# perrysou/SoftGNSS-python

Hardware: NVIDIA B200
Metric: tracking channel-ms/s (higher is better)
Workload: dtype int8 x Q38 fixed-point correlators (exact int32 dot products), f64 rotors / accumulation / loop filters

## Files before the change

### softgnss_python_b200/csrc/sgx_common.cuh

```cuda
#pragma once
#include <stdint.h>
#include <stdio.h>
#include <string.h>
#include <mutex>

#ifdef SGX_EMUL
#include "cuda_emul.h"
#else
#include <cuda_runtime.h>
#define SGX_LAUNCH(kernel, grid, block, smem, stream, ...) \
  kernel<<<(grid), (block), (smem), (stream)>>>(__VA_ARGS__)
#define SGX_DYN_SMEM(name) extern __shared__ __align__(1024) unsigned char name[]
#endif

#include "../../include/softgnss_b200.h"

#ifdef SGX_EMUL
#define SGX_TABLE static
#else
#define SGX_TABLE static __constant__
#endif

namespace sgx {

// ... 91 lines not shown

__device__ __forceinline__ void mbar_init(unsigned long long* bar, unsigned count) {
#ifdef SGX_EMUL
  *bar = 0;
  (void)count;
#else
  unsigned s = (unsigned)__cvta_generic_to_shared(bar);
  asm volatile("mbarrier.init.shared::cta.b64 [%0], %1;\n" ::"r"(s), "r"(count) : "memory");
  asm volatile("fence.mbarrier_init.release.cluster;\n" ::: "memory");
#endif
}
__device__ __forceinline__ unsigned smem_addr(const void* p) {
#ifdef SGX_EMUL
  (void)p; return 0u;
#else
  unsigned a = (unsigned)__cvta_generic_to_shared(p), o;
  asm volatile("mov.u32 %0, %1;" : "=r"(o) : "r"(a));
  return o;
#endif
}
__device__ __forceinline__ unsigned lds_u32(const void* base, unsigned base_s, int byte_off) {
#ifdef SGX_EMUL
  (void)base_s; return *reinterpret_cast<const unsigned*>(reinterpret_cast<const char*>(base) + byte_off);
#else
  (void)base; unsigned v;
  asm volatile("ld.shared.u32 %0, [%1];" : "=r"(v) : "r"(base_s + (unsigned)byte_off));
  return v;
#endif
}
__device__ __forceinline__ uint4 lds_u32x4(const void* base, unsigned base_s, int byte_off) {
#ifdef SGX_EMUL
  (void)base_s; return *reinterpret_cast<const uint4*>(reinterpret_cast<const char*>(base) + byte_off);
#else
  (void)base; uint4 v;
  asm volatile("ld.shared.v4.u32 {%0, %1, %2, %3}, [%4];" : "=r"(v.x), "=r"(v.y), "=r"(v.z), "=r"(v.w)
               : "r"(base_s + (unsigned)byte_off));
  return v;
#endif
}
__device__ __forceinline__ double2 lds_f64x2(const void* base, unsigned base_s, int byte_off) {
#ifdef SGX_EMUL
  (void)base_s; return *reinterpret_cast<const double2*>(reinterpret_cast<const char*>(base) + byte_off);
#else
  (void)base; double2 v;
  asm volatile("ld.shared.v2.f64 {%0, %1}, [%2];" : "=d"(v.x), "=d"(v.y) : "r"(base_s + (unsigned)byte_off));
  return v;
#endif
}

__device__ __forceinline__ void bulk_load(void* smem_dst, const void* gsrc, unsigned bytes,
                                          unsigned long long* bar) {
#ifdef SGX_EMUL
  memcpy(smem_dst, gsrc, bytes);
  *bar += 1;
#else
  unsigned d = (unsigned)__cvta_generic_to_shared(smem_dst);
  unsigned b = (unsigned)__cvta_generic_to_shared(bar);
  asm volatile("mbarrier.arrive.expect_tx.shared::cta.b64 _, [%0], %1;\n" ::"r"(b), "r"(bytes) : "memory");
  asm volatile(
      "cp.async.bulk.shared::cluster.global.mbarrier::complete_tx::bytes [%0], [%1], %2, [%3];\n" ::"r"(d),
      "l"(gsrc), "r"(bytes), "r"(b)
      : "memory");
#endif
}
__device__ __forceinline__ void mbar_wait(unsigned long long* bar, unsigned parity) {
#ifdef SGX_EMUL
  while ((*(volatile unsigned long long*)bar & 1ull) == (unsigned long long)parity) sgx_emul::yield_to_sched();
#else
  unsigned b = (unsigned)__cvta_generic_to_shared(bar);
  asm volatile(
      "{\n"
      ".reg .pred p;\n"
      "LAB_WAIT:\n"
      "mbarrier.try_wait.parity.shared::cta.b64 p, [%0], %1;\n"
      "@p bra DONE;\n"
      "bra LAB_WAIT;\n"
      "DONE:\n"
      "}\n" ::"r"(b),
      "r"(parity)
      : "memory");
#endif
}

__device__ __forceinline__ float warp_sum(float v) {
#pragma unroll
  for (int m = 16; m > 0; m >>= 1) v += __shfl_xor_sync(0xffffffffu, v, m);
  return v;
}

__device__ __forceinline__ double warp_sum_f64(double v) {
#pragma unroll
  for (int m = 16; m > 0; m >>= 1) v += __shfl_xor_sync(0xffffffffu, v, m);
  return v;
}

}
```

### softgnss_python_b200/csrc/sgx_track.cu

```cuda
#include <vector>
#include <fcntl.h>
#include <sys/stat.h>
#include <unistd.h>
#include "sgx_common.cuh"

namespace sgx {

constexpr int TRK_THREADS = 256;
constexpr int TRK_WARPS = TRK_THREADS / 32;
constexpr int TRK_MARGIN = 256;
constexpr int TRK_PROF_N = 5;

struct TrackArgs {
  const int8_t* rec;
  long long rec_stride;
  const long long* rec_len;
  const sgx_channel* ch;
  const int8_t* chips;
  double* out;
  int* ms_done;
  int* status;
  int n_channels;
  int ms;
  int resume;
  long long avail;
  struct TrackState* state;
  long long* prof;
  int win;
  long long skip;
  long long abs_base;
  double fs, codeFreqBasis, codeLength, spc;
  double c1code, c2code, c1carr, c2carr;
};

struct MsParams {
  double startE, stepE, startL, stepL, startP, stepP;
  double inv_step;
  long long q0_fix, h_fix;
  double cps;
  double rem_cyc;
  double w;
  double rem_rad;
  double fs;
  long long pos;
  int blk;
  int stop;
};

__device__ __forceinline__ double lin_y(int i, double step, double start) {
  return __dadd_rn(__dmul_rn((double)i, step), start);
}

__device__ __forceinline__ int next_event(int c, double start, double step, double inv) {
  double q = ((double)c - start) * inv;
  double fl = floor(q);
  int i = (int)fl + 1;
  double fr = q - fl;
  if (fr < 1e-6 || fr > 1.0 - 1e-6) {
    while (i > 0 && lin_y(i - 1, step, start) > (double)c) --i;
    while (!(lin_y(i, step, start) > (double)c)) ++i;
  }
  return i;
}

struct CodeVar {
  double start, step;
  int c;
  int e;
  float s;
  __device__ __forceinline__ void init(int i0, double st, double sp, double inv, const float* code) {
    start = st;
    step = sp;
    c = (int)ceil(lin_y(i0, step, start));
    s = code[c];
    e = next_event(c, start, step, inv);
  }
  __device__ __forceinline__ void advance(double inv, const float* code) {
    c += 1;
    s = code[c];
    e = next_event(c, start, step, inv);
  }
};

__device__ __forceinline__ float byte_to_float(unsigned u_offset_binary, int k) {
  unsigned r = __byte_perm(u_offset_binary, 0x4B000000u, 0x7540u + (unsigned)k);
  return __uint_as_float(r) - 8388736.0f;
}

__device__ __forceinline__ void cis_cycles(double cyc, float& c, float& s) {
  cyc -= rint(cyc);
  const float hi = (float)cyc;
  const float lo = (float)(cyc - (double)hi) * 6.2831853071795865f;
  float s0, c0;
  sincospif(2.0f * hi, &s0, &c0);
  c = fmaf(-s0, lo, c0);
  s = fmaf(c0, lo, s0);
}

__device__ __forceinline__ void cmul(float& r, float& i, float ar, float ai, float br, float bi) {
  r = fmaf(ar, br, -(ai * bi));
  i = fmaf(ar, bi, ai * br);
}

struct CodeState {
  double codeFreq, remCodePhase, oldCodeNco, oldCodeError, nextRemCode;
  long long pos;
};
struct CarrState {
  double carrFreq, carrFreqBasis, remCarrPhase, oldCarrNco, oldCarrError, w;
};

constexpr int SGX_PAUSED = 1;

struct TrackState {
  CodeState c;
  CarrState r;
  int k;
  int status;
};

__device__ void prepare_code(const TrackArgs& a, CodeState& st, long long rec_len, MsParams& p, int lane) {
  const double step = st.codeFreq / a.fs;
  const double q = (lane == 1 ? 1.0 : a.codeLength - st.remCodePhase) / step;
  const int blk = (int)ceil(__shfl_sync(0xffffffffu, q, 0));
  const double inv_step = __shfl_sync(0xffffffffu, q, 1);
  const long long aligned = st.pos & ~15LL;
  int stop = 0;
  if (st.pos + blk > rec_len) stop = SGX_ERR_SHORT;
  else if (st.pos + blk > a.avail) stop = SGX_PAUSED;
  else if (blk <= 0 || (st.pos - aligned) + blk > a.win) stop = SGX_ERR_RANGE;
  if (lane == 0) { p.blk = blk; p.pos = st.pos; p.stop = stop; }
  if (stop) return;
  const double rem = st.remCodePhase, spc = a.spc, bs = (double)blk * step;
  const double startE = rem - spc, startL = rem + spc, startP = rem;
  const double num = lane == 0 ? ((bs + rem) - spc) - startE : lane == 1 ? ((bs + rem) + spc) - startL : (bs + rem) - startP;
  const double d = num / (double)blk;
  const double stepE = __shfl_sync(0xffffffffu, d, 0), stepL = __shfl_sync(0xffffffffu, d, 1),
               stepP = __shfl_sync(0xffffffffu, d, 2);
  if (lane == 0) {
    p.startE = startE; p.stepE = stepE;
    p.startL = startL; p.stepL = stepL;
    p.startP = startP; p.stepP = stepP;
    p.inv_step = inv_step;
    p.h_fix = __double2ll_rn(0.5 * inv_step * 1099511627776.0);
    p.q0_fix = __double2ll_rn(-rem * inv_step * 1099511627776.0);
  }
  st.nextRemCode = (lin_y(blk - 1, stepP, startP) + step) - 1023.0;
}

__device__ double prepare_carr(const TrackArgs& a, CarrState& st, MsParams& p, bool write) {
  st.w = st.carrFreq * 2.0 * 3.141592653589793;
  const double cps = (st.w / a.fs) * 0.15915494309189535;
  if (write) {
    p.cps = cps;
    p.w = st.w;
    p.fs = a.fs;
  }
  return cps;
}

__device__ __forceinline__ void set_carr_phase(MsParams& p, double rem) {
  p.rem_cyc = rem * 0.15915494309189535;
  p.rem_rad = rem;
}

__device__ double carry_carr_phase(double w, double rem, int blk, double fs) {
  const double TWO_PI = 6.283185307179586;
  double arg_end = w * ((double)blk / fs) + rem;
  double m;
  if (arg_end >= 0.0) {
    double q = floor(arg_end * 0.15915494309189535);
    m = __fma_rn(-q, TWO_PI, arg_end);
    if (m < 0.0) { q -= 1.0; m = __fma_rn(-q, TWO_PI, arg_end); }
    else if (m >= TWO_PI) { q += 1.0; m = __fma_rn(-q, TWO_PI, arg_end); }
  } else {
    m = fmod(arg_end, TWO_PI);
    if (m != 0.0 && m < 0.0) m += TWO_PI;
  }
  return m;
}

__device__ __forceinline__ void correlate_groups(const MsParams& P, const int8_t* cur, const float* codeS, int tid,
                                                 double& tEr, double& tEi, double& tPr, double& tPi, double& tLr,
                                                 double& tLi) {
    const int off = (int)(P.pos - (P.pos & ~15LL));
    const int ng = (off + P.blk + 15) >> 4;
    const int gpt = (ng + TRK_THREADS - 1) / TRK_THREADS;
    const int g0 = tid * gpt;
    const int g1 = min(g0 + gpt, ng);
    if (g0 < g1) {
      int ib = 16 * g0 - off;
      const int i0 = max(ib, 0);
      CodeVar E, Pm, L;
      E.init(i0, P.startE, P.stepE, P.inv_step, codeS);
      Pm.init(i0, P.startP, P.stepP, P.inv_step, codeS);
      L.init(i0, P.startL, P.stepL, P.inv_step, codeS);
      float wr[16], wi[16], w16r, w16i, rotr, roti;
      {
        cis_cycles((double)ib * P.cps + P.rem_cyc, rotr, roti);
        float s1, c1;
        cis_cycles(P.cps, c1, s1);
        wr[0] = 1.f; wi[0] = 0.f; wr[1] = c1; wi[1] = s1;
#pragma unroll
        for (int q = 2; q < 16; ++q) {
          cmul(wr[q], wi[q], wr[q >> 1], wi[q >> 1], wr[q - (q >> 1)], wi[q - (q >> 1)]);
        }
        cis_cycles(16.0 * P.cps, w16r, w16i);
      }
      for (int g = g0; g < g1; ++g, ib += 16) {
        uint4 q4 = *reinterpret_cast<const uint4*>(cur + 16 * g);
        unsigned wq[4] = {q4.x, q4.y, q4.z, q4.w};
        if (ib < 0 || ib + 16 > P.blk) {
#pragma unroll
          for (int b = 0; b < 16; ++b) {
            int i = ib + b;
            if (i < 0 || i >= P.blk) wq[b >> 2] &= ~(0xFFu << (8 * (b & 3)));
          }
        }
#pragma unroll
        for (int j = 0; j < 4; ++j) wq[j] ^= 0x80808080u;
        const int kE = E.e - ib, kP = Pm.e - ib, kL = L.e - ib;
// ... 175 lines not shown
        cmul(tr, ti, cr, ci, zr[4], zi[4]);
        cr = tr; ci = ti;
      }
    }
    float Rr, Ri;
    cmul(Rr, Ri, rotr, roti, Sr, Si);
    fEr = fmaf(sE, Rr, fEr); fEi = fmaf(sE, Ri, fEi);
    fPr = fmaf(sP, Rr, fPr); fPi = fmaf(sP, Ri, fPi);
    fLr = fmaf(sL, Rr, fLr); fLi = fmaf(sL, Ri, fLi);
    const int len = b - a0;
    const int j = len - (LMAX - 4);
    if (j >= 0 && j <= 4) {
      float sr = zr[0], si = zi[0];
      if (j == 1) { sr = zr[1]; si = zi[1]; }
      if (j == 2) { sr = zr[2]; si = zi[2]; }
      if (j == 3) { sr = zr[3]; si = zi[3]; }
      if (j == 4) { sr = zr[4]; si = zi[4]; }
      float nr, ni;
      cmul(nr, ni, rotr, roti, sr, si);
      rotr = nr; roti = ni;
    } else {
      fresh = true;
    }
  }
  tEr += (double)fEr; tEi += (double)fEi; tPr += (double)fPr; tPi += (double)fPi; tLr += (double)fLr; tLi += (double)fLi;
}

template <int NW> struct ExactDigits { static constexpr int value = NW <= 5 ? 5 : 4; };
struct __align__(16) ExactTables {
  signed char tw[2][5][32];
  double z[5][2];
};

__device__ __forceinline__ void sincos_reduced(double th, double& sn, double& cs) {
  const double k = rint(th * 0.6366197723675814);
  double r = fma(-k, 1.5707963267341256, th);
  r = fma(-k, 6.077100506303966e-11, r);
  r = fma(-k, 2.0222662487959506e-21, r);
  const double r2 = r * r;
  double ps = -7.647163731819816e-13;
  ps = fma(ps, r2, 1.6059043836821613e-10);
  ps = fma(ps, r2, -2.505210838544172e-08);
  ps = fma(ps, r2, 2.7557319223985893e-06);
  ps = fma(ps, r2, -1.984126984126984e-04);
  ps = fma(ps, r2, 8.333333333333333e-03);
  ps = fma(ps, r2, -1.6666666666666666e-01);
  const double s0 = fma(ps * r2, r, r);
  double pc = 4.779477332387385e-14;
  pc = fma(pc, r2, -1.1470745597729725e-11);
  pc = fma(pc, r2, 2.08767569878681e-09);
  pc = fma(pc, r2, -2.755731922398589e-07);
  pc = fma(pc, r2, 2.48015873015873e-05);
  pc = fma(pc, r2, -1.388888888888889e-03);
  pc = fma(pc, r2, 4.1666666666666664e-02);
  pc = fma(pc, r2, -0.5);
  const double c0 = fma(pc, r2, 1.0);
  const int q = (int)(long long)k & 3;
  const double sa = (q & 1) ? c0 : s0, ca = (q & 1) ? s0 : c0;
  sn = (q & 2) ? -sa : sa;
  cs = ((q + 1) & 2) ? -ca : ca;
}

__device__ __forceinline__ void cis_cycles_f64(double cyc, double& c, double& s) {
  cyc -= rint(cyc);
  sincospi(2.0 * cyc, &s, &c);
}

template <int NW>
__device__ __forceinline__ void build_exact_tables(ExactTables& T, double cps, int lane) {
  constexpr int LMAX = 4 * NW;
  constexpr int ND = ExactDigits<NW>::value;
  constexpr int Z0 = (LMAX + 5 <= 32) ? LMAX : 0;
  const bool tw = lane < LMAX, zs = lane >= Z0 && lane < Z0 + 5;
  if (tw || (Z0 > 0 && zs)) {
    double c, s;
    cis_cycles_f64((double)(tw ? lane : LMAX - 4 + (lane - Z0)) * cps, c, s);
    if (!tw) {
      T.z[lane - Z0][0] = c;
      T.z[lane - Z0][1] = s;
      return;
    }
    const double one = (double)(1LL << (8 * ND - 2));
    long long w[2] = {__double2ll_rn(c * one), __double2ll_rn(s * one)};
#pragma unroll
    for (int q = 0; q < 2; ++q) {
      long long v = w[q];
#pragma unroll
      for (int d = 0; d < ND - 1; ++d) {
        const long long b = ((v + 128) & 0xFF) - 128;
        T.tw[q][d][lane] = (signed char)b;
        v = (v - b) >> 8;
      }
      T.tw[q][ND - 1][lane] = (signed char)v;
    }
  }
  if (Z0 == 0 && zs) cis_cycles_f64((double)(LMAX - 4 + lane) * cps, T.z[lane][0], T.z[lane][1]);
}

constexpr int IRREGULAR = 1 << 30;
__device__ __noinline__ int settle_boundary(int n, const MsParams& P) {
  if ((n & 1) == 0) return max(0, min(next_event(n >> 1, P.startP, P.stepP, P.inv_step), P.blk));
  const int c = (n - 1) >> 1;
  const int b = next_event(c, P.startE, P.stepE, P.inv_step);
  const int bl = next_event(c + 1, P.startL, P.stepL, P.inv_step);
  return max(0, min(b, P.blk)) | (bl != b ? IRREGULAR : 0);
}

__device__ __noinline__ double2 start_rotor(int a, const MsParams& P) {
  const double th = P.w * ((double)a / P.fs) + P.rem_rad;
  double sn, cs;
  if (fabs(th) < 5.0e5) sincos_reduced(th, sn, cs);
  else sincos(th, &sn, &cs);
  return make_double2(cs, sn);
}

__device__ __noinline__ void correlate_per_sample(const MsParams& P, const int8_t* cur, const unsigned char* codeB, int off,
                                                  int i0, int i1, double* acc) {
  for (int i = i0; i < i1; ++i) {
    const int ie = (int)ceil(lin_y(i, P.stepE, P.startE));
    const int ip = (int)ceil(lin_y(i, P.stepP, P.startP));
    const int il = (int)ceil(lin_y(i, P.stepL, P.startL));
    double cs, sn;
    cis_cycles_f64((double)i * P.cps + P.rem_cyc, cs, sn);
    const double x = (double)cur[off + i];
    const double pr = x * cs, pi = x * sn;
    const double ce = codeB[ie] ? -1.0 : 1.0, cp = codeB[ip] ? -1.0 : 1.0, cl = codeB[il] ? -1.0 : 1.0;
    acc[0] += ce * pr; acc[1] += ce * pi;
    acc[2] += cp * pr; acc[3] += cp * pi;
    acc[4] += cl * pr; acc[5] += cl * pi;
  }
}

__device__ __forceinline__ double flip_sign(double x, unsigned m) {
  return __hiloint2double(__double2hiint(x) ^ (int)m, __double2loint(x));
}

__device__ __forceinline__ double digits_to_double(int lo, int mid, int hi) {
  long long v = (long long)mid * 65536 + (long long)lo;
  v += (long long)hi << 32;
  v += 0x4338000000000000LL;
  return __longlong_as_double(v) - 6755399441055744.0;
}

template <int NW, int SEGS>
__device__ __forceinline__ void correlate_exact(const MsParams& P, const MsParams& Pcold, const int8_t* cur,
                                                const unsigned char* codeB, const ExactTables& T, int tid,
                                                double& tEr, double& tEi, double& tPr, double& tPi, double& tLr,
                                                double& tLi) {
  constexpr int LMAX = 4 * NW;
  constexpr int ND = ExactDigits<NW>::value;
  static_assert(SEGS == 8, "sign bytes are fetched for 8 half-chip segments per thread");
  const int off = (int)(P.pos - (P.pos & ~15LL));
  const int n0 = SEGS * tid - 1;
  const long long FR_ONE = 1LL << 40, FR_EPS = 1099512;
  long long qf = P.q0_fix + (long long)n0 * P.h_fix;
  auto boundary = [&](int n, long long q) -> int {
    if (n < 0) return 0;
    if (n > 2046) return P.blk;
    const long long fr = q & (FR_ONE - 1);
    if (fr < FR_EPS || fr > FR_ONE - FR_EPS) return settle_boundary(n, Pcold);
    return max(0, min((int)(q >> 40) + 1, P.blk));
  };
  int a = boundary(n0, qf);
  if ((a & ~IRREGULAR) >= P.blk) return;
  int s0 = 0;
  if (n0 < 0) {
    const int b0 = boundary(0, qf + P.h_fix);
    if ((b0 & ~IRREGULAR) == (a & ~IRREGULAR)) { s0 = 1; qf += P.h_fix; a = b0; }
  }
  int twr[ND][NW], twi[ND][NW];
#pragma unroll
  for (int d = 0; d < ND; ++d)
#pragma unroll
    for (int q = 0; q < NW; ++q) {
      twr[d][q] = reinterpret_cast<const int*>(T.tw[0][d])[q];
      twi[d][q] = reinterpret_cast<const int*>(T.tw[1][d])[q];
// ... 4 lines not shown
  double aEr = 0, aEi = 0, aPr = 0, aPi = 0, aLr = 0, aLi = 0;
  bool fresh = true;
  const unsigned cur_s = smem_addr(cur), z_s = smem_addr(&T.z[0][0]);
#pragma unroll 1
  for (int s = s0; s < SEGS; ++s) {
    qf += P.h_fix;
    const int b = boundary(n0 + s + 1, qf);
    const int len = (b & ~IRREGULAR) - (a & ~IRREGULAR);
    if (len > 0) {
      if (len > LMAX || ((a | b) & IRREGULAR)) {
        double acc[6] = {0, 0, 0, 0, 0, 0};
        correlate_per_sample(Pcold, cur, codeB, off, a & ~IRREGULAR, b & ~IRREGULAR, acc);
        const double up = (double)(1LL << (8 * ND - 2));
        aEr += acc[0] * up; aEi += acc[1] * up; aPr += acc[2] * up; aPi += acc[3] * up; aLr += acc[4] * up; aLi += acc[5] * up;
        fresh = true;
      } else {
        const unsigned mE = sg_lo << 24, mL = __byte_perm(sg_lo, 0u, 0x1444), mP = (s & 1) ? mL : mE;
        if (fresh) {
          const double2 r0 = start_rotor(a, Pcold);
          rotr = r0.x; roti = r0.y;
          fresh = false;
        }
        const int sh = ((off + a) & 3) * 8;
        unsigned raw[NW + 1];
        {
          constexpr int NQ = (NW + 7) / 4;
          const int ab = (off + a) & ~15, j = ((off + a) >> 2) & 3;
          unsigned wd[4 * NQ];
#pragma unroll
          for (int q = 0; q < NQ; ++q) {
            uint4 v = make_uint4(0u, 0u, 0u, 0u);
            if (q < NQ - 1 || j + NW >= 4 * (NQ - 1)) v = lds_u32x4(cur, cur_s, ab + 16 * q);
            wd[4 * q] = v.x; wd[4 * q + 1] = v.y; wd[4 * q + 2] = v.z; wd[4 * q + 3] = v.w;
          }
          unsigned t[NW + 2];
#pragma unroll
          for (int q = 0; q < NW + 2; ++q) t[q] = (j & 2) ? wd[q + 2] : wd[q];
#pragma unroll
          for (int q = 0; q <= NW; ++q) raw[q] = (j & 1) ? t[q + 1] : t[q];
        }
        unsigned w[NW];
#pragma unroll
        for (int q = 0; q < NW; ++q) w[q] = __funnelshift_r(raw[q], raw[q + 1], sh);
        w[NW - 1] &= __funnelshift_lc(0xFFFFFFFFu, 0u, max(8 * (len - 4 * (NW - 1)), 0));
        if (len < LMAX - 4) {
#pragma unroll
          for (int q = 0; q < NW - 1; ++q) w[q] &= __funnelshift_lc(0xFFFFFFFFu, 0u, max(8 * (len - 4 * q), 0));
        }
        int xr[ND], xi[ND];
#pragma unroll
        for (int d = 0; d < ND; ++d) { xr[d] = 0; xi[d] = 0; }
#pragma unroll
        for (int q = 0; q < NW; ++q) {
#pragma unroll
          for (int d = 0; d < ND; ++d) {
            xr[d] = __dp4a((int)w[q], twr[d][q], xr[d]);
            xi[d] = __dp4a((int)w[q], twi[d][q], xi[d]);
          }
        }
        const double Sr = digits_to_double(xr[1] * 256 + xr[0], xr[3] * 256 + xr[2], ND == 5 ? xr[ND - 1] : 0);
        const double Si = digits_to_double(xi[1] * 256 + xi[0], xi[3] * 256 + xi[2], ND == 5 ? xi[ND - 1] : 0);
        const double Rr = fma(rotr, Sr, -(roti * Si)), Ri = fma(rotr, Si, roti * Sr);
        aEr += flip_sign(Rr, mE); aEi += flip_sign(Ri, mE);
        aPr += flip_sign(Rr, mP); aPi += flip_sign(Ri, mP);
        aLr += flip_sign(Rr, mL); aLi += flip_sign(Ri, mL);
        const int j = len - (LMAX - 4);
        if (j >= 0) {
          const double2 z = lds_f64x2(&T.z[0][0], z_s, 16 * j);
          const double zr = z.x, zi = z.y;
          const double nr = fma(rotr, zr, -(roti * zi)), ni = fma(rotr, zi, roti * zr);
          rotr = nr; roti = ni;
        } else {
          fresh = true;
        }
      }
    }
    a = b;
    if (s & 1) { sg_lo = __funnelshift_r(sg_lo, sg_hi, 8); sg_hi >>= 8; }
  }
  const double sc = 1.0 / (double)(1LL << (8 * ND - 2));
  tEr += aEr * sc; tEi += aEi * sc; tPr += aPr * sc; tPi += aPi * sc; tLr += aLr * sc; tLi += aLi * sc;
}

template <bool BULK, int NW, bool EXACT, int NT>
__global__ void __launch_bounds__(NT, 2) track_kernel(TrackArgs a) {
  SGX_DYN_SMEM(smem);
  int8_t* buf0 = (int8_t*)smem;
  int8_t* buf1 = buf0 + a.win;
  __shared__ MsParams prm;
  constexpr int NWARPS = NT / 32;
  __shared__ double red[NWARPS][6];
  __shared__ float codeS[1040];
  __shared__ unsigned long long mbar[2];
  __shared__ ExactTables xt;
  __shared__ CodeState cstS;
  __shared__ CarrState rstS;
  __shared__ __align__(4) unsigned char codeB[EXACT ? 1040 : 4];
  __shared__ long long stampS[NWARPS][TRK_PROF_N + 1];
  __shared__ double remNextS;

  const int tid = threadIdx.x;
  const int lane = tid & 31;
  const int cid = blockIdx.x;
  const int rid = cid / a.n_channels;
  const sgx_channel chn = a.ch[cid];
  if (chn.prn == 0) {
    if (tid == 0) {
      a.ms_done[cid] = 0;
      a.status[cid] = SGX_OK;
      if (a.state) { a.state[cid].k = 0; a.state[cid].status = SGX_OK; }
    }
    return;
  }
  const int8_t* rec = a.rec + (long long)rid * a.rec_stride;
  const long long rec_len = a.rec_len[rid];
  const long long rec_alloc = (rec_len + 15) & ~15LL;
  {
    const int8_t* c = a.chips + (chn.prn - 1) * 1023;
    for (int i = tid; i < 1040; i += NT) {
      codeS[i] = i < 1025 ? (float)c[(i + 1022) % 1023] : 0.f;
      if (EXACT) codeB[i] = codeS[i] < 0.f ? 0x80 : 0;
    }
  }
  int k_start = 0;
  if (a.resume) {
    const TrackState* ts = a.state + cid;
    if (ts->status != SGX_PAUSED) return;
    k_start = ts->k;
    if (tid < 32) { CodeState c = ts->c; prepare_code(a, c, rec_len, prm, lane); if (lane == 0) cstS = c; }
    if (tid == 32) { CarrState r = ts->r; prepare_carr(a, r, prm, true); set_carr_phase(prm, r.remCarrPhase); rstS = r; }
    if (tid == 0 && BULK) { mbar_init(&mbar[0], 1); mbar_init(&mbar[1], 1); }
  } else {
    if (tid < 32) {
      CodeState c;
      c.codeFreq = a.codeFreqBasis;
      c.remCodePhase = 0.0;
      c.oldCodeNco = c.oldCodeError = 0.0;
      c.nextRemCode = 0.0;
      c.pos = a.skip + (long long)chn.codePhase;
      prepare_code(a, c, rec_len, prm, lane);
      if (lane == 0) cstS = c;
    }
    if (tid == 0 && BULK) { mbar_init(&mbar[0], 1); mbar_init(&mbar[1], 1); }
    if (tid == 32) {
      CarrState r;
      r.carrFreq = chn.acquiredFreq;
      r.carrFreqBasis = chn.acquiredFreq;
      r.remCarrPhase = 0.0;
      r.oldCarrNco = r.oldCarrError = 0.0;
      prepare_carr(a, r, prm, true);
      set_carr_phase(prm, r.remCarrPhase);
      rstS = r;
    }
  }
  if (EXACT && (tid >> 5) == 1) {
    const double cps = __shfl_sync(0xffffffffu, tid == 32 ? prm.cps : 0.0, 0);
    build_exact_tables<(NW > 0 ? NW : 1)>(xt, cps, tid & 31);
  }
  __syncthreads();

  auto stage = [&](int8_t* dst, long long pos) {
    long long al = pos & ~15LL;
    long long nb = rec_alloc - al;
    if (nb > a.win) nb = a.win;
    if (nb <= 0) return 0;
    if (BULK) {
      return (int)nb;
    } else {
      const int8_t* src = rec + al;
      for (int o = tid * 16; o < (int)nb; o += NT * 16) cp_async16(dst + o, src + o);
      cp_async_commit();
      return (int)nb;
    }
  };
  unsigned phase0 = 0, phase1 = 0;
  bool pending0 = false, pending1 = false;
  if (prm.stop == 0) {
    const int par = k_start & 1;
    int nb = stage(par ? buf1 : buf0, prm.pos);
    if (BULK) {
      if (nb > 0) {
        if (tid == 0) bulk_load(par ? buf1 : buf0, rec + (prm.pos & ~15LL), (unsigned)nb, &mbar[par]);
        if (par) pending1 = true; else pending0 = true;
      }
      const long long npos = prm.pos + prm.blk;
      const int nb1 = stage(par ? buf0 : buf1, npos);
      if (tid == 0 && nb1 > 0 && k_start < a.ms) bulk_load(par ? buf0 : buf1, rec + (npos & ~15LL), (unsigned)nb1, &mbar[par ^ 1]);
    }
  }

  int k = k_start;
  for (; k < a.ms; ++k) {
    const MsParams P = prm;
    if (P.stop != 0) break;
    const bool stamp = a.prof && (tid & 31) == 0;
    long long* ts = stampS[tid >> 5];
    if (stamp) ts[0] = clock64();
    int8_t* cur = (k & 1) ? buf1 : buf0;
    int8_t* nxt = (k & 1) ? buf0 : buf1;
    if (BULK) {
      if (k & 1) { if (pending1) { mbar_wait(&mbar[1], phase1); phase1 ^= 1; pending1 = false; } }
      else       { if (pending0) { mbar_wait(&mbar[0], phase0); phase0 ^= 1; pending0 = false; } }
    } else {
      if (k == k_start) { cp_async_wait_all(); __syncthreads(); }
    }
    {
      long long npos = P.pos + P.blk;
      int nb = stage(nxt, npos);
      if (BULK && nb > 0) {
        if (k & 1) pending0 = true; else pending1 = true;
      }
    }
    if (tid == 64) remNextS = carry_carr_phase(P.w, P.rem_rad, P.blk, P.fs);
    if (stamp) ts[1] = clock64();

    double tEr = 0.0, tEi = 0.0, tPr = 0.0, tPi = 0.0, tLr = 0.0, tLi = 0.0;
    if (EXACT)       correlate_exact<(NW > 0 ? NW : 1), 2048 / NT>(P, prm, cur, codeB, xt, tid, tEr, tEi, tPr, tPi, tLr, tLi);
    else if (NW > 0) correlate_segments<(NW > 0 ? NW : 1)>(P, cur, codeS, tid, tEr, tEi, tPr, tPi, tLr, tLi);
    else             correlate_groups(P, cur, codeS, tid, tEr, tEi, tPr, tPi, tLr, tLi);
    if (stamp) ts[2] = clock64();
    double v0 = warp_sum_f64(tEi), v1 = warp_sum_f64(tEr), v2 = warp_sum_f64(tPi), v3 = warp_sum_f64(tPr),
           v4 = warp_sum_f64(tLi), v5 = warp_sum_f64(tLr);
    if ((tid & 31) == 0) {
      double* r = red[tid >> 5];
      r[0] = v0; r[1] = v1; r[2] = v2; r[3] = v3; r[4] = v4; r[5] = v5;
    }
    if (!BULK) cp_async_wait_all();
    __syncthreads();
    if (stamp) ts[3] = clock64();
    if (tid < 32) {
      CodeState cst = cstS;
      const int blk = prm.blk;
      __syncwarp();
      double I_E = 0.0, Q_E = 0.0, I_L = 0.0, Q_L = 0.0;
      for (int w = 0; w < NWARPS; ++w) { I_E += red[w][0]; Q_E += red[w][1]; I_L += red[w][4]; Q_L += red[w][5]; }
      cst.remCodePhase = cst.nextRemCode;
      cst.pos = cst.pos + blk;
      const double mag = sqrt(lane == 1 ? I_L * I_L + Q_L * Q_L : I_E * I_E + Q_E * Q_E);
      const double em = __shfl_sync(0xffffffffu, mag, 0), lm = __shfl_sync(0xffffffffu, mag, 1);
      double codeError = (em - lm) / (em + lm);
      double codeNco = cst.oldCodeNco + a.c1code * (codeError - cst.oldCodeError) + codeError * a.c2code;
      cst.oldCodeNco = codeNco;
      cst.oldCodeError = codeError;
      cst.codeFreq = a.codeFreqBasis - codeNco;
      if (k + 1 < a.ms) prepare_code(a, cst, rec_len, prm, lane);
      if (lane == 0) {
        cstS = cst;
        if (BULK && k + 1 < a.ms && prm.stop == 0) {
          const long long npos = prm.pos + prm.blk;
          const int nb = stage(cur, npos);
          if (nb > 0) bulk_load(cur, rec + (npos & ~15LL), (unsigned)nb, &mbar[k & 1]);
        }
        double* o = a.out + (long long)cid * SGX_TRACK_FIELDS * a.ms + k;
        const long long m = a.ms;
        o[0 * m] = (double)(cst.pos + a.abs_base);
        o[1 * m] = cst.codeFreq;
        o[4 * m] = I_E; o[5 * m] = I_L; o[6 * m] = Q_E; o[8 * m] = Q_L;
        o[9 * m] = codeError; o[10 * m] = codeNco;
      }
    } else if (tid < 64) {
      CarrState rst = rstS;
      __syncwarp();
      double I_P = 0.0, Q_P = 0.0;
      for (int w = 0; w < NWARPS; ++w) { I_P += red[w][2]; Q_P += red[w][3]; }
      double carrError = atan(Q_P / I_P) * 0.5 / 3.141592653589793;
      double carrNco = rst.oldCarrNco + a.c1carr * (carrError - rst.oldCarrError) + carrError * a.c2carr;
      rst.oldCarrNco = carrNco;
      rst.oldCarrError = carrError;
      rst.carrFreq = rst.carrFreqBasis + carrNco;
      if (k + 1 < a.ms) {
        const double cps = prepare_carr(a, rst, prm, lane == 0);
        if (EXACT) build_exact_tables<(NW > 0 ? NW : 1)>(xt, cps, lane);
      }
      if (lane == 0) {
        double* o = a.out + (long long)cid * SGX_TRACK_FIELDS * a.ms + k;
        const long long m = a.ms;
        o[2 * m] = rst.carrFreq;
        o[3 * m] = I_P; o[7 * m] = Q_P;
        o[11 * m] = carrError; o[12 * m] = carrNco;
        rstS = rst;
      }
    } else if (tid == 64) {
      set_carr_phase(prm, remNextS);
    }
    if (stamp) ts[4] = clock64();
    __syncthreads();
    if (stamp) {
      ts[5] = clock64();
      long long* pr = a.prof + ((long long)cid * NWARPS + (tid >> 5)) * TRK_PROF_N;
#pragma unroll
      for (int i = 0; i < TRK_PROF_N; ++i) pr[i] += ts[i + 1] - ts[i];
    }
  }
  if (BULK) {
    if (pending0) mbar_wait(&mbar[0], phase0);
    if (pending1) mbar_wait(&mbar[1], phase1);
  } else {
    cp_async_wait_all();
  }
  if (tid == 0) {
    const int status = (k == a.ms) ? SGX_OK : prm.stop;
    a.ms_done[cid] = k;
    a.status[cid] = status;
    if (a.state) { a.state[cid].c = cstS; a.state[cid].k = k; a.state[cid].status = status; }
  }
  if (tid == 32 && a.state) {
    CarrState r = rstS;
    r.remCarrPhase = prm.rem_rad;
    a.state[cid].r = r;
  }
}

struct TrackScratch {
  DevBuf rec, len, ch, chips, out, done, status, state, prof;
  cudaStream_t copy_stream = nullptr;
  cudaEvent_t ev[2] = {nullptr, nullptr};
  int8_t* pin[2] = {nullptr, nullptr};
  size_t pin_cap = 0;
  cudaEvent_t pin_ev[2] = {nullptr, nullptr};
};

struct FileSrc {
  int fd;
  int sample_bytes;
  long long base;
  long long len;
  long long chunk;
  int bad_value;
};
static TrackScratch g_trk;

static bool use_bulk() {
  const char* e = getenv("SGX_TRK_STAGE");
  return !(e && strcmp(e, "cpasync") == 0);
}

}

using namespace sgx;

static int track_core(const int8_t* rec, int64_t rec_stride, const int64_t* rec_len,
                      int32_t n_recordings, const sgx_channel* ch, int32_t n_channels,
                      const sgx_settings* st, const int8_t* ca_chips, double* out,
                      int32_t* ms_done, void* cuda_stream, sgx::FileSrc* file) {
  if ((!rec && !file) || !rec_len || !ch || !st || !ca_chips || !out || !ms_done || n_recordings <= 0 ||
      n_channels <= 0 || st->msToProcess <= 0)
    return fail(SGX_ERR_ARG, "sgx_track", "null pointer or empty problem");
  const int nch = n_recordings * n_channels;
  for (int i = 0; i < nch; ++i)
    if (ch[i].prn < 0 || ch[i].prn > SGX_NUM_PRN) return fail(SGX_ERR_ARG, "sgx_track", "PRN outside 0..32");
  cudaStream_t s = (cudaStream_t)cuda_stream;
  const int ms = st->msToProcess;
  const int win = ((st->samplesPerCode + TRK_MARGIN + 15) & ~15) + 16;

  const int8_t* d_rec = rec;
  long long stride = rec_stride;
  long long max_len = 0;
  for (int r = 0; r < n_recordings; ++r) max_len = rec_len[r] > max_len ? rec_len[r] : max_len;
  const bool host_input = file || !is_device_ptr(rec);
  if (host_input) {
    stride = (max_len + 15) & ~15LL;
    if (g_trk.rec.reserve((size_t)stride * n_recordings + 16)) return fail(SGX_ERR_CUDA, "cudaMalloc", "recording");
    d_rec = g_trk.rec.as<int8_t>();
  } else if (((rec_stride & 15) && n_recordings > 1) || ((uintptr_t)rec & 15)) {
    return fail(SGX_ERR_ARG, "sgx_track", "device recordings must be 16-byte aligned with a stride multiple of 16");
  }
  if (g_trk.len.reserve(sizeof(long long) * n_recordings) || g_trk.ch.reserve(sizeof(sgx_channel) * nch) ||
      g_trk.chips.reserve(32 * 1023) || g_trk.done.reserve(sizeof(int) * nch) ||
      g_trk.status.reserve(sizeof(int) * nch) || g_trk.state.reserve(sizeof(TrackState) * nch))
    return fail(SGX_ERR_CUDA, "cudaMalloc", "tracking scratch");
  SGX_CUDA(cudaMemcpyAsync(g_trk.len.p, rec_len, sizeof(long long) * n_recordings, cudaMemcpyHostToDevice, s));
  SGX_CUDA(cudaMemcpyAsync(g_trk.ch.p, ch, sizeof(sgx_channel) * nch, cudaMemcpyHostToDevice, s));
  SGX_CUDA(cudaMemcpyAsync(g_trk.chips.p, ca_chips, 32 * 1023, cudaMemcpyHostToDevice, s));
  const size_t out_bytes = sizeof(double) * (size_t)nch * SGX_TRACK_FIELDS * ms;
  double* d_out = out;
  const bool out_on_host = !is_device_ptr(out);
  if (out_on_host) {
    if (g_trk.out.reserve(out_bytes)) return fail(SGX_ERR_CUDA, "cudaMalloc", "tracking output");
    d_out = g_trk.out.as<double>();
  }

  TrackArgs a;
  a.rec = d_rec;
  a.rec_stride = stride;
  a.rec_len = g_trk.len.as<long long>();
  a.ch = g_trk.ch.as<sgx_channel>();
  a.chips = g_trk.chips.as<int8_t>();
  a.out = d_out;
  a.ms_done = g_trk.done.as<int>();
  a.status = g_trk.status.as<int>();
  a.n_channels = n_channels;
  a.ms = ms;
  a.resume = 0;
  a.avail = 0x7fffffffffffffffLL;
  a.state = g_trk.state.as<TrackState>();
  a.prof = nullptr;
  const size_t prof_n = (size_t)nch * TRK_WARPS * TRK_PROF_N;
  if (getenv("SGX_TRK_PROF")) {
    if (g_trk.prof.reserve(sizeof(long long) * prof_n)) return fail(SGX_ERR_CUDA, "cudaMalloc", "prof");
    SGX_CUDA(cudaMemsetAsync(g_trk.prof.p, 0, sizeof(long long) * prof_n, s));
    a.prof = g_trk.prof.as<long long>();
  }
  a.win = win;
  a.skip = file ? st->skipNumberOfBytes / file->sample_bytes - file->base : st->skipNumberOfBytes;
  a.abs_base = file ? file->base : 0;
  a.fs = st->samplingFreq;
  a.codeFreqBasis = st->codeFreqBasis;
  a.codeLength = (double)st->codeLength;
  a.spc = st->dllCorrelatorSpacing;
  a.c1code = st->tau2code / st->tau1code;
  a.c2code = st->PDIcode / st->tau1code;
  a.c1carr = st->tau2carr / st->tau1carr;
  a.c2carr = st->PDIcarr / st->tau1carr;

  const size_t smem = 2 * (size_t)win;
  auto launch = [&]() -> int {
  const double half_chip = st->samplingFreq / (2.0 * st->codeFreqBasis);
  int nw = ((int)ceil(half_chip + 0.25) + 3) / 4;
  bool exact = true;
  if (const char* e = getenv("SGX_TRK_KERNEL")) {
    if (strcmp(e, "groups") == 0) nw = 0;
    if (strcmp(e, "segments") == 0) exact = false;
  }
  if (fabs(st->dllCorrelatorSpacing - 0.5) > 1e-12) nw = 0;
  const bool bulk = use_bulk();
#define SGX_TRK_GO_NT(B, W, X, NTHR)                                                               \
  {                                                                                                \
    auto kfn = track_kernel<B, W, X, NTHR>;                                                        \
    SGX_CUDA(cudaFuncSetAttribute(kfn, cudaFuncAttributeMaxDynamicSharedMemorySize, (int)smem));   \
    SGX_COUNTED_LAUNCH(kfn, dim3(nch), dim3(NTHR), smem, s, a);                                    \
  }
#define SGX_TRK_GO(B, W, X) SGX_TRK_GO_NT(B, W, X, TRK_THREADS)
#define SGX_TRK_EXACT(W) { if (bulk) SGX_TRK_GO(true, W, true) else SGX_TRK_GO(false, W, true) }
  if (nw >= 1 && nw <= 8 && exact) {
    switch (nw) {
      case 1: SGX_TRK_EXACT(1) break;
      case 2: SGX_TRK_EXACT(2) break;
      case 3: SGX_TRK_EXACT(3) break;
      case 4: SGX_TRK_EXACT(4) break;
      case 5: SGX_TRK_EXACT(5) break;
      case 6: SGX_TRK_EXACT(6) break;
      case 7: SGX_TRK_EXACT(7) break;
      default: SGX_TRK_EXACT(8) break;
    }
  } else if (nw == 5) {
    if (bulk) SGX_TRK_GO(true, 5, false) else SGX_TRK_GO(false, 5, false)
  } else {
    if (bulk) SGX_TRK_GO(true, 0, false) else SGX_TRK_GO(false, 0, false)
  }
#undef SGX_TRK_EXACT
#undef SGX_TRK_GO
#undef SGX_TRK_GO_NT
    return SGX_OK;
  };
  if (!host_input) {
    int rc0 = launch();
    if (rc0) return rc0;
  } else {
    if (!g_trk.copy_stream) {
      SGX_CUDA(cudaStreamCreateWithFlags(&g_trk.copy_stream, cudaStreamNonBlocking));
      SGX_CUDA(cudaEventCreateWithFlags(&g_trk.ev[0], cudaEventDisableTiming));
      SGX_CUDA(cudaEventCreateWithFlags(&g_trk.ev[1], cudaEventDisableTiming));
    }
    long long chunk = 1024LL * st->samplesPerCode;
    if (const char* e = getenv("SGX_TRK_CHUNK_MS")) { if (atoll(e) > 0) chunk = atoll(e) * st->samplesPerCode; }
    chunk = (chunk + 15) & ~15LL;
    SGX_CUDA(cudaEventRecord(g_trk.ev[1], s));
    SGX_CUDA(cudaStreamWaitEvent(g_trk.copy_stream, g_trk.ev[1], 0));
    int c = 0;
    if (file) chunk = file->chunk;
    for (long long off = 0; off < max_len; off += chunk, ++c) {
      const long long width = (max_len - off) < chunk ? (max_len - off) : chunk;
      if (file) {
        int8_t* hb = g_trk.pin[c & 1];
        if (c >= 2) SGX_CUDA(cudaEventSynchronize(g_trk.pin_ev[c & 1]));
        const size_t bytes = (size_t)width * file->sample_bytes;
        size_t got = 0;
        while (got < bytes) {
          const ssize_t r = pread(file->fd, (char*)hb + got, bytes - got, (off_t)((file->base + off) * file->sample_bytes + (long long)got));
          if (r <= 0) return fail(SGX_ERR_ARG, "sgx_track_file", "short read from the recording file");
          got += (size_t)r;
        }
        if (file->sample_bytes == 2) {
          const int16_t* src = (const int16_t*)hb;
          for (long long i = 0; i < width; ++i) {
            const int v = src[i];
            if (v < -128 || v > 127) file->bad_value = 1;
            hb[i] = (int8_t)v;
          }
          if (file->bad_value) return fail(SGX_ERR_ARG, "sgx_track_file", "int16 sample outside the int8 range of the correlators");
        }
        SGX_CUDA(cudaMemcpyAsync(g_trk.rec.as<int8_t>() + off, hb, (size_t)width, cudaMemcpyHostToDevice, g_trk.copy_stream));
        SGX_CUDA(cudaEventRecord(g_trk.pin_ev[c & 1], g_trk.copy_stream));
      } else
      SGX_CUDA(cudaMemcpy2DAsync(g_trk.rec.as<int8_t>() + off, (size_t)stride, rec + off, (size_t)rec_stride, (size_t)width,
                                 (size_t)n_recordings, cudaMemcpyHostToDevice, g_trk.copy_stream));
      SGX_CUDA(cudaEventRecord(g_trk.ev[0], g_trk.copy_stream));
      SGX_CUDA(cudaStreamWaitEvent(s, g_trk.ev[0], 0));
      a.avail = off + width;
      a.resume = c > 0;
      int rc0 = launch();
      if (rc0) return rc0;
    }
  }
  SGX_CUDA(cudaGetLastError());
  if (out_on_host) SGX_CUDA(cudaMemcpyAsync(out, d_out, out_bytes, cudaMemcpyDeviceToHost, s));
  std::vector<int> h_status_v(nch);
  int* h_status = h_status_v.data();
  SGX_CUDA(cudaMemcpyAsync(ms_done, a.ms_done, sizeof(int) * nch, cudaMemcpyDeviceToHost, s));
  SGX_CUDA(cudaMemcpyAsync(h_status, a.status, sizeof(int) * nch, cudaMemcpyDeviceToHost, s));
  SGX_CUDA(cudaStreamSynchronize(s));
  if (a.prof) {
    std::vector<long long> hp(prof_n);
    cudaMemcpy(hp.data(), a.prof, sizeof(long long) * prof_n, cudaMemcpyDeviceToHost);
    const double per = (double)nch * ms;
    fprintf(stderr, "[sgx prof] cycles/period  warp:  wait+prefetch  correlate  reduce+bar  bookkeeping  bar  | period\n");
    for (int w = 0; w < TRK_WARPS; ++w) {
      double acc[TRK_PROF_N] = {}, tot = 0.0;
      for (int i = 0; i < nch; ++i)
        for (int j = 0; j < TRK_PROF_N; ++j) acc[j] += (double)hp[((size_t)i * TRK_WARPS + w) * TRK_PROF_N + j];
      for (int j = 0; j < TRK_PROF_N; ++j) tot += acc[j];
      fprintf(stderr, "[sgx prof] %d: %8.0f %8.0f %8.0f %8.0f %8.0f | %8.0f\n", w, acc[0] / per, acc[1] / per, acc[2] / per,
              acc[3] / per, acc[4] / per, tot / per);
    }
  }
  int rc = SGX_OK;
  for (int i = 0; i < nch; ++i)
    if (h_status[i] != SGX_OK && rc == SGX_OK) rc = h_status[i];
  if (rc == SGX_ERR_SHORT) return fail(rc, "sgx_track", "Not able to read the specified number of samples for tracking");
  if (rc != SGX_OK) return fail(rc, "sgx_track", "loop state left the supported range");
  return SGX_OK;
}

extern "C" int sgx_track(const int8_t* rec, int64_t rec_stride, const int64_t* rec_len,
                         int32_t n_recordings, const sgx_channel* ch, int32_t n_channels,
                         const sgx_settings* st, const int8_t* ca_chips, double* out,
                         int32_t* ms_done, void* cuda_stream) {
  if (sgx_device_count() <= 0) return fail(SGX_ERR_NODEV, "sgx_track", "no CUDA device");
  SGX_API_GUARD();
  return track_core(rec, rec_stride, rec_len, n_recordings, ch, n_channels, st, ca_chips, out, ms_done, cuda_stream,
                    nullptr);
}

extern "C" int sgx_track_file(const char* path, int32_t sample_bytes, const sgx_channel* ch, int32_t n_channels,
                              const sgx_settings* st, const int8_t* ca_chips, double* out, int32_t* ms_done,
                              int64_t chunk_samples, int64_t* window ,
                              void* cuda_stream) {
  if (sgx_device_count() <= 0) return fail(SGX_ERR_NODEV, "sgx_track_file", "no CUDA device");
  SGX_API_GUARD();
  if (!path || !ch || !st || n_channels <= 0 || (sample_bytes != 1 && sample_bytes != 2))
    return fail(SGX_ERR_ARG, "sgx_track_file", "null pointer, or dataType other than int8 / int16");
  const int fd = open(path, O_RDONLY);
  if (fd < 0) return fail(SGX_ERR_ARG, "sgx_track_file", "cannot open the recording file");
  struct stat sb;
  if (fstat(fd, &sb) != 0) { close(fd); return fail(SGX_ERR_ARG, "sgx_track_file", "cannot stat the recording file"); }
  const long long file_samples = (long long)sb.st_size / sample_bytes;
  double cp_min = 1e300, cp_max = -1e300;
  for (int i = 0; i < n_channels; ++i)
    if (ch[i].prn > 0) { cp_min = ch[i].codePhase < cp_min ? ch[i].codePhase : cp_min; cp_max = ch[i].codePhase > cp_max ? ch[i].codePhase : cp_max; }
  if (cp_max < cp_min) { cp_min = cp_max = 0.0; }
  const long long skip = st->skipNumberOfBytes / sample_bytes;
  FileSrc fs;
  fs.fd = fd;
  fs.sample_bytes = sample_bytes;
  fs.bad_value = 0;
  fs.base = (skip + (long long)cp_min) & ~15LL;
  const double need = (double)(skip + (long long)cp_max - fs.base) + ((double)st->msToProcess * (1.0 + 1e-4) + 2.0) * st->samplesPerCode + 64.0;
  fs.len = file_samples - fs.base;
  if (fs.len > (long long)need) fs.len = (long long)need;
  if (fs.len <= 0) { close(fd); return fail(SGX_ERR_SHORT, "sgx_track_file", "Not able to read the specified number of samples for tracking"); }
  fs.chunk = chunk_samples > 0 ? chunk_samples : 1024LL * st->samplesPerCode;
  fs.chunk = (fs.chunk + 15) & ~15LL;
  const size_t pin_bytes = (size_t)fs.chunk * sample_bytes;
  if (g_trk.pin_cap < pin_bytes) {
    for (int i = 0; i < 2; ++i) {
      if (g_trk.pin[i]) cudaFreeHost(g_trk.pin[i]);
      g_trk.pin[i] = nullptr;
      if (cudaHostAlloc((void**)&g_trk.pin[i], pin_bytes, cudaHostAllocDefault) != cudaSuccess) {
        g_trk.pin_cap = 0;
        close(fd);
        return fail(SGX_ERR_CUDA, "cudaHostAlloc", "pinned staging buffers");
      }
      if (!g_trk.pin_ev[i]) cudaEventCreateWithFlags(&g_trk.pin_ev[i], cudaEventDisableTiming);
    }
    g_trk.pin_cap = pin_bytes;
  }
  if (window) { window[0] = fs.base; window[1] = fs.len; }
  const int64_t rec_len = fs.len;
  const int rc = track_core(nullptr, 0, &rec_len, 1, ch, n_channels, st, ca_chips, out, ms_done, cuda_stream, &fs);
  close(fd);
  return rc;
}
```

Baseline: 37.02 million.

## Combine six warp reductions into one shuffle tree and refine profiling

Replaces six separate butterfly warp sums with one combined transposed shuffle reduction, so fewer shuffles are needed before the per-warp partials go to shared memory. Simplifies the twiddle digit decomposition into a bias-and-extract form with no serial carry chain. Moves the code-loop output stores ahead of prepare_code. Profiling now accumulates in shared memory, records finer sub-stage timestamps, SM id and global time, and can dump per-CTA data. The new profiling is gated by an environment variable.

New measurement: 36.80 million (median of 6 runs). About the same (-0.6%).

```diff
diff --git a/softgnss_python_b200/csrc/sgx_common.cuh b/softgnss_python_b200/csrc/sgx_common.cuh
--- a/softgnss_python_b200/csrc/sgx_common.cuh
+++ b/softgnss_python_b200/csrc/sgx_common.cuh
@@ -197,6 +197,25 @@
 #endif
 }
 
+__device__ __forceinline__ int sm_id() {
+#ifdef SGX_EMUL
+  return 0;
+#else
+  int v;
+  asm volatile("mov.u32 %0, %%smid;" : "=r"(v));
+  return v;
+#endif
+}
+__device__ __forceinline__ long long global_ns() {
+#ifdef SGX_EMUL
+  return 0;
+#else
+  long long v;
+  asm volatile("mov.u64 %0, %%globaltimer;" : "=l"(v));
+  return v;
+#endif
+}
+
 __device__ __forceinline__ float warp_sum(float v) {
 #pragma unroll
   for (int m = 16; m > 0; m >>= 1) v += __shfl_xor_sync(0xffffffffu, v, m);
diff --git a/softgnss_python_b200/csrc/sgx_track.cu b/softgnss_python_b200/csrc/sgx_track.cu
--- a/softgnss_python_b200/csrc/sgx_track.cu
+++ b/softgnss_python_b200/csrc/sgx_track.cu
@@ -10,6 +10,9 @@
 constexpr int TRK_WARPS = TRK_THREADS / 32;
 constexpr int TRK_MARGIN = 256;
 constexpr int TRK_PROF_N = 5;
+constexpr int TRK_SUB_N = 6;
+constexpr int TRK_PROF_W = TRK_PROF_N + TRK_SUB_N;
+constexpr int TRK_CTA_N = 6;
 
 struct TrackArgs {
   const int8_t* rec;
@@ -119,7 +122,8 @@
   int status;
 };
 
-__device__ void prepare_code(const TrackArgs& a, CodeState& st, long long rec_len, MsParams& p, int lane) {
+__device__ void prepare_code(const TrackArgs& a, CodeState& st, long long rec_len, MsParams& p, int lane,
+                             long long* ts = nullptr) {
   const double step = st.codeFreq / a.fs;
   const double q = (lane == 1 ? 1.0 : a.codeLength - st.remCodePhase) / step;
   const int blk = (int)ceil(__shfl_sync(0xffffffffu, q, 0));
@@ -130,6 +134,7 @@
   else if (st.pos + blk > a.avail) stop = SGX_PAUSED;
   else if (blk <= 0 || (st.pos - aligned) + blk > a.win) stop = SGX_ERR_RANGE;
   if (lane == 0) { p.blk = blk; p.pos = st.pos; p.stop = stop; }
+  if (ts) ts[0] = clock64();
   if (stop) return;
   const double rem = st.remCodePhase, spc = a.spc, bs = (double)blk * step;
   const double startE = rem - spc, startL = rem + spc, startP = rem;
@@ -137,6 +142,7 @@
   const double d = num / (double)blk;
   const double stepE = __shfl_sync(0xffffffffu, d, 0), stepL = __shfl_sync(0xffffffffu, d, 1),
                stepP = __shfl_sync(0xffffffffu, d, 2);
+  if (ts) ts[1] = clock64();
   if (lane == 0) {
     p.startE = startE; p.stepE = stepE;
     p.startL = startL; p.stepL = stepL;
@@ -478,16 +484,13 @@
     }
     const double one = (double)(1LL << (8 * ND - 2));
     long long w[2] = {__double2ll_rn(c * one), __double2ll_rn(s * one)};
+    constexpr long long BIAS = (1LL << (8 * (ND - 1))) / 255 * 128;
 #pragma unroll
     for (int q = 0; q < 2; ++q) {
-      long long v = w[q];
-#pragma unroll
-      for (int d = 0; d < ND - 1; ++d) {
-        const long long b = ((v + 128) & 0xFF) - 128;
-        T.tw[q][d][lane] = (signed char)b;
-        v = (v - b) >> 8;
-      }
-      T.tw[q][ND - 1][lane] = (signed char)v;
+      const long long u = w[q] + BIAS;
+#pragma unroll
+      for (int d = 0; d < ND - 1; ++d) T.tw[q][d][lane] = (signed char)(((unsigned)(u >> (8 * d)) & 0xFFu) ^ 0x80u);
+      T.tw[q][ND - 1][lane] = (signed char)(u >> (8 * (ND - 1)));
     }
   }
   if (Z0 == 0 && zs) cis_cycles_f64((double)(LMAX - 4 + lane) * cps, T.z[lane][0], T.z[lane][1]);
@@ -658,6 +661,19 @@
   tEr += aEr * sc; tEi += aEi * sc; tPr += aPr * sc; tPi += aPi * sc; tLr += aLr * sc; tLi += aLi * sc;
 }
 
+__device__ __forceinline__ double warp_sum6(double v0, double v1, double v2, double v3, double v4, double v5, int lane) {
+  const bool h16 = lane & 16, h8 = lane & 8, h4 = lane & 4;
+  const double a = (h16 ? v3 : v0) + __shfl_xor_sync(0xffffffffu, h16 ? v0 : v3, 16);
+  const double b = (h16 ? v4 : v1) + __shfl_xor_sync(0xffffffffu, h16 ? v1 : v4, 16);
+  const double c = (h16 ? v5 : v2) + __shfl_xor_sync(0xffffffffu, h16 ? v2 : v5, 16);
+  const double f = (h8 ? c : a) + __shfl_xor_sync(0xffffffffu, h8 ? a : c, 8);
+  const double g = b + __shfl_xor_sync(0xffffffffu, b, 8);
+  double v = (!h8 && h4 ? g : f) + __shfl_xor_sync(0xffffffffu, (h8 || h4) ? f : g, 4);
+  v += __shfl_xor_sync(0xffffffffu, v, 2);
+  v += __shfl_xor_sync(0xffffffffu, v, 1);
+  return v;
+}
+
 template <bool BULK, int NW, bool EXACT, int NT>
 __global__ void __launch_bounds__(NT, 2) track_kernel(TrackArgs a) {
   SGX_DYN_SMEM(smem);
@@ -672,7 +688,9 @@
   __shared__ CodeState cstS;
   __shared__ CarrState rstS;
   __shared__ __align__(4) unsigned char codeB[EXACT ? 1040 : 4];
-  __shared__ long long stampS[NWARPS][TRK_PROF_N + 1];
+  __shared__ long long stampS[NWARPS][TRK_PROF_N + 1 + TRK_SUB_N];
+  __shared__ long long accS[NWARPS][TRK_PROF_W];
+  __shared__ long long startS[2];
   __shared__ double remNextS;
 
   const int tid = threadIdx.x;
@@ -687,6 +705,10 @@
       if (a.state) { a.state[cid].k = 0; a.state[cid].status = SGX_OK; }
     }
     return;
+  }
+  if (a.prof) {
+    if (tid == 0) { startS[0] = clock64(); startS[1] = global_ns(); }
+    if (tid < NWARPS * TRK_PROF_W) accS[tid / TRK_PROF_W][tid % TRK_PROF_W] = 0;
   }
   const int8_t* rec = a.rec + (long long)rid * a.rec_stride;
   const long long rec_len = a.rec_len[rid];
@@ -795,11 +817,9 @@
     else if (NW > 0) correlate_segments<(NW > 0 ? NW : 1)>(P, cur, codeS, tid, tEr, tEi, tPr, tPi, tLr, tLi);
     else             correlate_groups(P, cur, codeS, tid, tEr, tEi, tPr, tPi, tLr, tLi);
     if (stamp) ts[2] = clock64();
-    double v0 = warp_sum_f64(tEi), v1 = warp_sum_f64(tEr), v2 = warp_sum_f64(tPi), v3 = warp_sum_f64(tPr),
-           v4 = warp_sum_f64(tLi), v5 = warp_sum_f64(tLr);
-    if ((tid & 31) == 0) {
-      double* r = red[tid >> 5];
-      r[0] = v0; r[1] = v1; r[2] = v2; r[3] = v3; r[4] = v4; r[5] = v5;
+    {
+      const double v = warp_sum6(tEi, tEr, tPi, tPr, tLi, tLr, lane);
+      if ((lane & 3) == 0 && (lane & 12) != 12) red[tid >> 5][(lane >> 4) * 3 + ((lane >> 2) & 3)] = v;
     }
     if (!BULK) cp_async_wait_all();
     __syncthreads();
@@ -810,16 +830,28 @@
       __syncwarp();
       double I_E = 0.0, Q_E = 0.0, I_L = 0.0, Q_L = 0.0;
       for (int w = 0; w < NWARPS; ++w) { I_E += red[w][0]; Q_E += red[w][1]; I_L += red[w][4]; Q_L += red[w][5]; }
+      long long* sub = ts + TRK_PROF_N + 1;
+      if (stamp) sub[0] = clock64();
       cst.remCodePhase = cst.nextRemCode;
       cst.pos = cst.pos + blk;
       const double mag = sqrt(lane == 1 ? I_L * I_L + Q_L * Q_L : I_E * I_E + Q_E * Q_E);
       const double em = __shfl_sync(0xffffffffu, mag, 0), lm = __shfl_sync(0xffffffffu, mag, 1);
       double codeError = (em - lm) / (em + lm);
+      if (stamp) sub[1] = clock64();
       double codeNco = cst.oldCodeNco + a.c1code * (codeError - cst.oldCodeError) + codeError * a.c2code;
       cst.oldCodeNco = codeNco;
       cst.oldCodeError = codeError;
       cst.codeFreq = a.codeFreqBasis - codeNco;
-      if (k + 1 < a.ms) prepare_code(a, cst, rec_len, prm, lane);
+      if (lane == 0) {
+        double* o = a.out + (long long)cid * SGX_TRACK_FIELDS * a.ms + k;
+        const long long m = a.ms;
+        o[0 * m] = (double)(cst.pos + a.abs_base);
+        o[1 * m] = cst.codeFreq;
+        o[4 * m] = I_E; o[5 * m] = I_L; o[6 * m] = Q_E; o[8 * m] = Q_L;
+        o[9 * m] = codeError; o[10 * m] = codeNco;
+      }
+      if (stamp) sub[2] = sub[3] = sub[4] = clock64();
+      if (k + 1 < a.ms) prepare_code(a, cst, rec_len, prm, lane, stamp ? sub + 3 : nullptr);
       if (lane == 0) {
         cstS = cst;
         if (BULK && k + 1 < a.ms && prm.stop == 0) {
@@ -827,26 +859,27 @@
           const int nb = stage(cur, npos);
           if (nb > 0) bulk_load(cur, rec + (npos & ~15LL), (unsigned)nb, &mbar[k & 1]);
         }
-        double* o = a.out + (long long)cid * SGX_TRACK_FIELDS * a.ms + k;
-        const long long m = a.ms;
-        o[0 * m] = (double)(cst.pos + a.abs_base);
-        o[1 * m] = cst.codeFreq;
-        o[4 * m] = I_E; o[5 * m] = I_L; o[6 * m] = Q_E; o[8 * m] = Q_L;
-        o[9 * m] = codeError; o[10 * m] = codeNco;
-      }
+      }
+      if (stamp) sub[5] = clock64();
     } else if (tid < 64) {
       CarrState rst = rstS;
       __syncwarp();
       double I_P = 0.0, Q_P = 0.0;
       for (int w = 0; w < NWARPS; ++w) { I_P += red[w][2]; Q_P += red[w][3]; }
+      long long* sub = ts + TRK_PROF_N + 1;
+      if (stamp) sub[0] = clock64();
       double carrError = atan(Q_P / I_P) * 0.5 / 3.141592653589793;
+      if (stamp) sub[1] = clock64();
       double carrNco = rst.oldCarrNco + a.c1carr * (carrError - rst.oldCarrError) + carrError * a.c2carr;
       rst.oldCarrNco = carrNco;
       rst.oldCarrError = carrError;
       rst.carrFreq = rst.carrFreqBasis + carrNco;
+      if (stamp) sub[2] = sub[3] = clock64();
       if (k + 1 < a.ms) {
         const double cps = prepare_carr(a, rst, prm, lane == 0);
+        if (stamp) sub[2] = clock64();
         if (EXACT) build_exact_tables<(NW > 0 ? NW : 1)>(xt, cps, lane);
+        if (stamp) sub[3] = clock64();
       }
       if (lane == 0) {
         double* o = a.out + (long long)cid * SGX_TRACK_FIELDS * a.ms + k;
@@ -863,9 +896,11 @@
     __syncthreads();
     if (stamp) {
       ts[5] = clock64();
-      long long* pr = a.prof + ((long long)cid * NWARPS + (tid >> 5)) * TRK_PROF_N;
-#pragma unroll
-      for (int i = 0; i < TRK_PROF_N; ++i) pr[i] += ts[i + 1] - ts[i];
+      long long* acc = accS[tid >> 5];
+#pragma unroll
+      for (int i = 0; i < TRK_PROF_N; ++i) acc[i] += ts[i + 1] - ts[i];
+      const int nsub = tid == 0 ? 6 : tid == 32 ? 4 : 0;
+      for (int i = 0; i < nsub; ++i) acc[TRK_PROF_N + i] += ts[TRK_PROF_N + 1 + i] - ts[i == 0 ? 3 : TRK_PROF_N + i];
     }
   }
   if (BULK) {
@@ -873,6 +908,21 @@
     if (pending1) mbar_wait(&mbar[1], phase1);
   } else {
     cp_async_wait_all();
+  }
+  if (a.prof && lane == 0) {
+    long long* pr = a.prof + ((long long)cid * NWARPS + (tid >> 5)) * TRK_PROF_W;
+    for (int i = 0; i < TRK_PROF_W; ++i) pr[i] += accS[tid >> 5][i];
+    if (tid == 0) {
+      long long* c = a.prof + (long long)gridDim.x * NWARPS * TRK_PROF_W + (long long)cid * TRK_CTA_N;
+      long long sum = 0;
+      for (int i = 0; i < TRK_PROF_N; ++i) sum += accS[0][i];
+      c[0] = sm_id();
+      c[1] = startS[0];
+      c[2] = clock64();
+      c[3] += sum;
+      c[4] = startS[1];
+      c[5] = global_ns();
+    }
   }
   if (tid == 0) {
     const int status = (k == a.ms) ? SGX_OK : prm.stop;
@@ -971,7 +1021,7 @@
   a.avail = 0x7fffffffffffffffLL;
   a.state = g_trk.state.as<TrackState>();
   a.prof = nullptr;
-  const size_t prof_n = (size_t)nch * TRK_WARPS * TRK_PROF_N;
+  const size_t prof_n = (size_t)nch * (TRK_WARPS * TRK_PROF_W + TRK_CTA_N);
   if (getenv("SGX_TRK_PROF")) {
     if (g_trk.prof.reserve(sizeof(long long) * prof_n)) return fail(SGX_ERR_CUDA, "cudaMalloc", "prof");
     SGX_CUDA(cudaMemsetAsync(g_trk.prof.p, 0, sizeof(long long) * prof_n, s));
@@ -1091,13 +1141,26 @@
     cudaMemcpy(hp.data(), a.prof, sizeof(long long) * prof_n, cudaMemcpyDeviceToHost);
     const double per = (double)nch * ms;
     fprintf(stderr, "[sgx prof] cycles/period  warp:  wait+prefetch  correlate  reduce+bar  bookkeeping  bar  | period\n");
+    double acc[TRK_WARPS][TRK_PROF_W] = {};
     for (int w = 0; w < TRK_WARPS; ++w) {
-      double acc[TRK_PROF_N] = {}, tot = 0.0;
+      double tot = 0.0;
       for (int i = 0; i < nch; ++i)
-        for (int j = 0; j < TRK_PROF_N; ++j) acc[j] += (double)hp[((size_t)i * TRK_WARPS + w) * TRK_PROF_N + j];
-      for (int j = 0; j < TRK_PROF_N; ++j) tot += acc[j];
-      fprintf(stderr, "[sgx prof] %d: %8.0f %8.0f %8.0f %8.0f %8.0f | %8.0f\n", w, acc[0] / per, acc[1] / per, acc[2] / per,
-              acc[3] / per, acc[4] / per, tot / per);
+        for (int j = 0; j < TRK_PROF_W; ++j) acc[w][j] += (double)hp[((size_t)i * TRK_WARPS + w) * TRK_PROF_W + j];
+      for (int j = 0; j < TRK_PROF_N; ++j) tot += acc[w][j];
+      fprintf(stderr, "[sgx prof] %d: %8.0f %8.0f %8.0f %8.0f %8.0f | %8.0f\n", w, acc[w][0] / per, acc[w][1] / per,
+              acc[w][2] / per, acc[w][3] / per, acc[w][4] / per, tot / per);
+    }
+    const double* s0 = acc[0] + TRK_PROF_N;
+    const double* s1 = acc[1] + TRK_PROF_N;
+    fprintf(stderr, "[sgx prof] code loop (warp 0):    red-sum %6.0f  sqrt+div %6.0f  filter+stores %6.0f  blk/step %6.0f  "
+            "slopes %6.0f  state+bulk %6.0f\n", s0[0] / per, s0[1] / per, s0[2] / per, s0[3] / per, s0[4] / per, s0[5] / per);
+    fprintf(stderr, "[sgx prof] carrier loop (warp 1): red-sum %6.0f  div+atan %6.0f  filter+stores+cps %6.0f  tables %6.0f\n",
+            s1[0] / per, s1[1] / per, s1[2] / per, s1[3] / per);
+    if (const char* path = getenv("SGX_TRK_PROF_CTA")) {
+      if (FILE* f = fopen(path, "wb")) {
+        fwrite(hp.data() + (size_t)nch * TRK_WARPS * TRK_PROF_W, sizeof(long long), (size_t)nch * TRK_CTA_N, f);
+        fclose(f);
+      }
     }
   }
   int rc = SGX_OK;
```
